# Stanford-ILIAD/PantheonRL

Hardware: AMD Instinct MI355X
Metric: env-steps/sec (all agents) Overcooked-simple PPO self-play (higher is better)
Workload: dtype f32; 1 GPU; OvercookedMultiEnv-v0 layout=simple, PPO self-play (two independent PPO learners per GPU), synthetic (n_envs, n_steps, obs_dim) rollouts; n_envs=1024, n_steps=128, obs_dim=62, features=62, n_logits=6, batch_size=32768, n_epochs=10, agents_per_gpu=2, parallelism=2 agent(s) per gpu x1 gpu(s) = 2 learners (single process), launch_mode=graph, gemm_mode=2, action_masks=none, rollout=scripted, rollout_requested=scripted

## Files before the change

pantheonrl_amd/csrc/ph_abi.hip:

```cpp
#include <dlfcn.h>
#include <hip/hip_runtime.h>
#include <rccl/rccl.h>

#include <atomic>
#include <chrono>
#include <cmath>
#include <cstdio>
#include <cstdint>
#include <cstring>
#include <mutex>
#include <string>
#include <vector>

#include "ph_launch.h"
#include "ph_block.h"
#include "ph_arch.h"
#include "ph_pool.h"

namespace ph {

namespace {
struct LdsGrant {
  const void* kernel;
  int device;
// ... 67 lines not shown
  int* slab_map_split = nullptr;
  int* wimage_map = nullptr;
  int split_kind = 0;
  int slab_len_split = 0;
  int wimage_elems = 0;
  int id = 0;
};

}

struct ph_ctx {
  int device = 0;
  hipStream_t stream = nullptr;
  float* slabs = nullptr;
  size_t slabs_cap = 0;
  float* statpart = nullptr;
  size_t statpart_cap = 0;
  float* grad = nullptr;
  size_t grad_cap = 0;
  float* blocksq = nullptr;
  size_t blocksq_cap = 0;
  float* advstats = nullptr;
  size_t advstats_cap = 0;
  float* act_stage_host = nullptr;
  float* act_stage_dev = nullptr;
  size_t act_stage_cap = 0;
  unsigned int* act_done_host = nullptr;
  unsigned int* act_done_dev = nullptr;
  unsigned int act_seq = 0;
  unsigned int* fwd_host_done = nullptr;
  int joint_reward_rule = 0;
  int wimage_zeroed_for = 0;
  size_t wimage_cap = 0;
  bool exclusive = false;
  unsigned short* wimage = nullptr;
  double* advpart = nullptr;
  size_t advpart_cap = 0;
  int* perm_idx = nullptr;
  size_t perm_idx_cap = 0;
  int* perm_phys = nullptr;
  size_t perm_phys_cap = 0;
  uint4* ximg = nullptr;
  size_t ximg_cap = 0;
  uint4* rec_pi = nullptr;
  uint4* rec_vf = nullptr;
  size_t rec_cap = 0;
// ... 540 lines not shown
    return fail("hipMalloc(ctx scalars) failed");
  }
  (void)hipMemset(c->scalars, 0, 4 * sizeof(float));
  (void)hipMemset(c->stop_flag, 0, sizeof(int));
  (void)hipEventCreate(&c->ev0);
  (void)hipEventCreate(&c->ev1);
  *out = c;
  return 0;
}

int ph_ctx_destroy(ph_ctx* ctx) {
  DevGuard dev_guard(ctx);
  if (!ctx) return 0;
  (void)hipStreamSynchronize(ctx->stream);
  for (auto g : ctx->graphs)
    if (g) (void)hipGraphExecDestroy(g);
  for (auto& s : ctx->specs) {
    if (s.obs_off) (void)hipFree(s.obs_off);
    if (s.slab_map) (void)hipFree(s.slab_map);
    if (s.slab_map_split) (void)hipFree(s.slab_map_split);
    if (s.wimage_map) (void)hipFree(s.wimage_map);
    if (s.act_off) (void)hipFree(s.act_off);
  }
  void* ptrs[] = {ctx->wimage, ctx->mw.act, ctx->mw.maps, ctx->mw.kl_sum, ctx->mw.scratch, ctx->advpart, ctx->p2p_dev, ctx->slabs, ctx->statpart, ctx->grad, ctx->blocksq, ctx->advstats, ctx->perm_idx, ctx->perm_phys, ctx->ximg, ctx->rec_pi, ctx->rec_vf, ctx->rowrec, ctx->step_words, ctx->step_gen, ctx->scalars, ctx->stop_flag,
                  ctx->adap_extra, ctx->adap_loss, ctx->am_buf, ctx->pool_dev, ctx->pool_order, ctx->pool_tiles};
  for (void* p : ptrs)
    if (p) (void)hipFree(p);
  if (ctx->act_stage_host) (void)hipHostFree(ctx->act_stage_host);
  if (ctx->act_done_host) (void)hipHostFree(ctx->act_done_host);
  if (ctx->ev0) (void)hipEventDestroy(ctx->ev0);
  if (ctx->ev1) (void)hipEventDestroy(ctx->ev1);
  if (ctx->ev_grad) (void)hipEventDestroy(ctx->ev_grad);
  (void)ph_comm_destroy(ctx);
  delete ctx;
  return 0;
}

int ph_ctx_set_joint_reward_rule(ph_ctx* ctx, int rule) {
  if (!ctx) return fail("null ctx");
  if (rule != PH_JOINT_MATCH_BONUS && rule != PH_JOINT_RPS) return fail("ph_ctx_set_joint_reward_rule: unknown rule");
  ctx->joint_reward_rule = rule;
  return 0;
}

int ph_ctx_set_stream(ph_ctx* ctx, void* hip_stream) {
  DevGuard dev_guard(ctx);
  if (!ctx) return fail("null ctx");
// ... 1418 lines not shown
  aa.rec_vf_out = nd.split == 1 ? ctx->rec_vf : nullptr;
  aa.rowrec = (nd.split == 1 && rb->advantages && rb->log_probs && rb->actions && rb->returns && rb->values) ? ctx->rowrec : nullptr;
  aa.rb_logp = rb->log_probs;
  aa.rb_act = rb->actions;
  aa.rb_ret = rb->returns;
  aa.rb_val = rb->values;
}


void select_gemm(ph::NetDims& nd, int gemm_mode) {
  nd.split = (gemm_mode == 2 && nd.slab_map_split != nullptr) ? nd.split_kind : 0;
  if (nd.split) nd.slab_map = nd.slab_map_split;
}

int slab_len_of(const ph::NetDims& nd) { return nd.split ? nd.slab_len_split : (nd.slab_map ? 2 * ph::RS_NET : nd.lay.P); }

int ensure_train_ws(ph_ctx* ctx, int P, int slab_len, int nwg_max, int n_mb_total, size_t n_idx = 0, size_t n_phys = 0) {
  if (n_phys && ensure(ctx, ctx->perm_phys, ctx->perm_phys_cap, n_phys)) return 1;
  if (ensure(ctx, ctx->slabs, ctx->slabs_cap, (size_t)nwg_max * slab_len)) return 1;
  if (ensure(ctx, ctx->statpart, ctx->statpart_cap, (size_t)2 * nwg_max * ph::NSTATP)) return 1;
  if (ensure(ctx, ctx->grad, ctx->grad_cap, (size_t)P)) return 1;
  if (ensure(ctx, ctx->blocksq, ctx->blocksq_cap, (size_t)ph::reduce_blocks(slab_len))) return 1;
  if (ensure(ctx, ctx->advstats, ctx->advstats_cap, (size_t)n_mb_total * 2)) return 1;
  if (ensure(ctx, ctx->advpart, ctx->advpart_cap, (size_t)n_mb_total * 2 * ph::ADV_SPLIT)) return 1;
  if (n_idx && ensure(ctx, ctx->perm_idx, ctx->perm_idx_cap, n_idx)) return 1;
  const size_t n_words = (size_t)ph::reduce_blocks(slab_len) + 1;
  if (n_words > ctx->step_words_cap) {
    if (ensure(ctx, ctx->step_words, ctx->step_words_cap, n_words)) return 1;
    PH_HIP(hipMemsetAsync(ctx->step_words, 0, n_words * sizeof(unsigned long long), ctx->stream));
  }
  if (!ctx->step_gen) {
    if (ctx->capturing) return fail("workspace would grow inside graph capture: run the same call once outside capture first");
    PH_HIP(hipMalloc((void**)&ctx->step_gen, 4 * sizeof(unsigned int)));
    PH_HIP(hipMemsetAsync(ctx->step_gen, 0, 4 * sizeof(unsigned int), ctx->stream));
  }
  return 0;
}

bool step_fused_wanted(const ph_ctx* ctx, int slab_len, bool alone) {
  return alone && ctx->exclusive && ctx->step_words && ctx->step_gen &&
         ph::step_fused_fits(ph::reduce_blocks(slab_len), slab_len, ctx->num_cu);
}

}

namespace {
// ... 63 lines not shown
  a.used_state_idx = ad->used_state_idx ? ad->used_state_idx + (size_t)mbi * S : nullptr;
  a.used_contexts = ad->used_contexts ? ad->used_contexts + (size_t)mbi * C * cs : nullptr;
  a.stop_flag = ctx->stop_flag;
  a.prof = ctx->prof;
  PH_HIP(ph::launch_adap_context(a, nwg, ctx->stream));
  r->extra = ctx->adap_extra;
  r->n_extra = nwg;
  r->extra_len = ph::adap_slab_floats(nd.lay);
  r->extra_cut = nd.lay.vf_W1;
  r->extra_lo = nd.lay.act_W;
  r->extra_hi = nd.lay.val_W;
  r->extra_loss = ctx->adap_loss;
  r->extra_norm = 1.0f / (float)((C * (C - 1) / 2) * n_states);
  r->extra_coef = ad->context_loss_coeff;
  r->extra_loss_out = ad->context_loss ? ad->context_loss + mbi : nullptr;
  return 0;
}

void train_adv_args(const TrainPlan& t, bool need_idx, ph::AdvStatArgs& aa) {
  aa = adv_args_epochs(t.ctx, t.rb, t.perms, t.perm_seed, t.batch_size, t.n_mb);
  aa.clear_flag = t.ctx->stop_flag;
  if (t.nd.split == 1 && !need_idx) aa.idx_out = aa.phys_out = nullptr;
  fill_adv_records(aa, t.ctx, t.nd, t.rb);
}

int train_prepare(const char* who, TrainPlan& t, ph_ctx* ctx, const ph_spec* spec, const ph_opt_state* opt, const ph_rollout* rb,
                  const ph_ppo_hyper* hp, int n_epochs, int batch_size, const int* perms, unsigned long long perm_seed,
                  float* stats, int gemm_mode, bool need_idx = false, const ph_arch* arch = nullptr) {
  if (check_train_call(who, ctx, opt, hp, n_epochs, batch_size) || check_rb(rb)) return 1;
  t.arch = arch != nullptr;
  if (arch) {
    if (arch_resolve(ctx, spec, arch, &t.nd, &t.arch_dims)) return 1;
  } else {
    if (resolve(ctx, spec, &t.nd, true)) return 1;
    select_gemm(t.nd, gemm_mode);
  }
  t.ctx = ctx;
  t.opt = opt;
  t.rb = rb;
  t.hp = hp;
  t.perms = perms;
  t.perm_seed = perm_seed;
  t.stats = stats;
  t.n_epochs = n_epochs;
  t.batch_size = batch_size;
  t.gemm_mode = gemm_mode;
// ... 32 lines not shown
    g.rec_vf = ctx->rec_vf + pos;
  }
  g.perm_n = (uint32_t)t.N;
  g.perm_hb = t.hb;
  g.perm_seed = t.perm_seed;
  g.perm_epoch = w.ep;
  g.epoch = ctx->rng_epoch;
  g.mb_start = w.start;
  g.nb = w.nb;
  g.advstats = ctx->advstats + 2 * (size_t)mbi;
  g.ntiles = pl.ntiles;
  *pl_out = pl;
  if (t.arch) PH_HIP(ph::launch_arch_grad(g, t.arch_dims, pl.nwg, t.gemm_mode, ctx->stream));
  else PH_HIP(ph::launch_ppo_grad(g, pl.nwg, t.gemm_mode, ctx->stream));
  return 0;
}

void fill_step_args(const TrainPlan& t, int mbi, const MbPlan& pl, ph::ReduceArgs& r, ph::AdamArgs& ad) {
  ph_ctx* ctx = t.ctx;
  float* stats_out = t.stats ? t.stats + (size_t)mbi * PH_NSTAT : nullptr;
  r = reduce_args(ctx, t.hp, t.opt, t.P, slab_len_of(t.nd), t.nd.slab_map, pl.nwg, pl.nb, ctx->grad, stats_out);
  r.wide = t.alone && ctx->exclusive;
  ad = adam_args(ctx, t.hp, t.opt, t.P, slab_len_of(t.nd), stats_out, t.nd.split ? ctx->wimage : nullptr, t.nd.wimage_map);
}

int train_launch_step(const TrainPlan& t, int mbi, const MbPlan& pl) {
  ph_ctx* ctx = t.ctx;
  hipStream_t s = ctx->stream;
  ph::ReduceArgs r;
  ph::AdamArgs ad;
  fill_step_args(t, mbi, pl, r, ad);
  if (t.adap) {
    const MbWalk w = minibatch_walk(ctx, t.perms, t.N, t.n_mb, t.batch_size, mbi);
    if (adap_launch(ctx, t.nd, t.opt->params, t.rb, t.adap, w.idx, w.nb, mbi, &r)) return 1;
  }
  if (step_fused_wanted(ctx, slab_len_of(t.nd), t.alone != 0)) {
    PH_HIP(ph::launch_ppo_step(r, ad, ctx->step_words, ctx->step_gen, ctx->step_gen + 1, STEP_WAIT_TICKS, s));
  } else {
    PH_HIP(ph::launch_ppo_reduce(r, s));
    PH_HIP(ph::launch_ppo_adam(ad, s));
  }
  return 0;
}

}

// ... 483 lines not shown
  auto timed = [&](int slot, auto&& fn) -> int {
    float ms = 0.f;
    if (time_reps(ctx, 1, reps, [&](int) { return fn(); }, &ms)) return 1;
    us_out[slot] = 1e3f * ms;
    return 0;
  };
  auto hip = [](hipError_t e) { return hip_rc(e, "ph_bench_train_kernels"); };
  if (t.nd.split) {
    if (timed(PH_BENCH_WEIGHT_IMAGE, [&] { return rebuild_weight_image(ctx, t.nd, opt->params); })) return 1;
    if (timed(PH_BENCH_OBS_PLANES, [&] { return build_grad_pack(ctx, t.nd, rb, (size_t)n_epochs * t.N); })) return 1;
  }
  ph::AdvStatArgs aa;
  train_adv_args(t, false, aa);
  if (timed(PH_BENCH_ADV_STATS, [&] { return hip(ph::launch_adv_stats(aa, n_epochs * t.n_mb, s)); })) return 1;
  MbPlan pl;
  if (train_launch_grad(t, 0, &pl)) return 1;
  ph::ReduceArgs r;
  ph::AdamArgs ad;
  fill_step_args(t, 0, pl, r, ad);
  r.wide = 0;
  if (timed(PH_BENCH_REDUCE, [&] { return hip(ph::launch_ppo_reduce(r, s)); })) return 1;
  r.wide = 1;
  if (timed(PH_BENCH_REDUCE_WIDE, [&] { return hip(ph::launch_ppo_reduce(r, s)); })) return 1;
  if (timed(PH_BENCH_ADAM, [&] { return hip(ph::launch_ppo_adam(ad, s)); })) return 1;
  if (ctx->step_words && ctx->step_gen && ph::step_fused_fits(ph::reduce_blocks(slab_len_of(t.nd)), slab_len_of(t.nd), ctx->num_cu)) {
    if (timed(PH_BENCH_STEP_FUSED, [&] {
          return hip(ph::launch_ppo_step(r, ad, ctx->step_words, ctx->step_gen, ctx->step_gen + 1, STEP_WAIT_TICKS, s));
        }))
      return 1;
  }
  if (rb->T >= 2) {
    const size_t E = (size_t)rb->E;
    if (timed(PH_BENCH_BUFFER_ADD, [&] {
          return hip(ph::launch_buffer_add(rb->observations + E * t.nd.D, rb->actions + E * t.nd.A, rb->rewards + E,
                                           rb->episode_starts + E, rb->values + E, rb->log_probs + E, rb->observations,
                                           rb->actions, rb->episode_starts, rb->values, rb->log_probs, rb->E, t.nd.D, t.nd.A, s));
        }))
      return 1;
  }
  us_out[PH_BENCH_SLAB_FLOATS] = (float)((double)pl.nwg * slab_len_of(t.nd));
  return 0;
}


namespace {

// ... 531 lines not shown
```

pantheonrl_amd/csrc/ph_launch.h:

```cpp
#pragma once
#include "ph_device.h"

namespace ph {

__host__ __device__ inline unsigned p2p_stamp32(unsigned long long epoch, int T, int t) {
  return (unsigned)(epoch * (unsigned long long)T + (unsigned long long)t + 1ull);
}

__device__ __forceinline__ void p2p_note_timeout(unsigned long long* error, int kind, int t, unsigned long long index,
                                                 unsigned long long want, unsigned long long seen) {
  if (atomicAdd(error, 1ull) == 0ull) {
    error[1] = (unsigned long long)(unsigned)kind | ((unsigned long long)(unsigned)(t & 0xffffff) << 8) | (index << 32);
    error[2] = want;
    error[3] = seen;
  }
}

__device__ __forceinline__ void poll_backoff(int& polls) {
  if (polls < 16) __builtin_amdgcn_s_sleep(2);
  else if (polls < 64) __builtin_amdgcn_s_sleep(16);
  else __builtin_amdgcn_s_sleep(127);
  ++polls;
}

// ... 117 lines not shown

__device__ __host__ inline uint64_t epoch_key(uint64_t seed, int epoch) {
  uint64_t z = seed + 0x9E3779B97F4A7C15ull * (uint64_t)(epoch + 1);
  z = (z ^ (z >> 30)) * 0xBF58476D1CE4E5B9ull;
  z = (z ^ (z >> 27)) * 0x94D049BB133111EBull;
  return z ^ (z >> 31);
}

__device__ __forceinline__ int env_major_to_phys(int n, int T, int E) {
  const int e = n / T;
  return (n - e * T) * E + e;
}
__device__ __forceinline__ int minibatch_row(const GradArgs& a, int gi) {
  int n;
  if (a.idx) {
    n = a.idx[gi];
  } else {
    const uint64_t key = epoch_key(a.perm_seed + (a.epoch ? *a.epoch : 0ull), a.perm_epoch);
    n = (int)feistel_perm((uint32_t)(a.mb_start + gi), a.perm_n, a.perm_hb, key);
  }
  return env_major_to_phys(n, a.T, a.E);
}

constexpr int ADV_SPLIT = 32;
constexpr int ADV_THREADS = 256;
struct AdvStatArgs {
  const float* rb_adv;
  int T, E;
  const int* perms;
  uint32_t perm_n, perm_hb;
  uint64_t perm_seed;
  const unsigned long long* epoch;
  int N, batch, n_mb;
  float* out;
  double* partial;
  int* idx_out;
  int* phys_out;
  uint4* rec_pi_out = nullptr;
  uint4* rec_vf_out = nullptr;
  const float *rb_logp = nullptr, *rb_act = nullptr, *rb_ret = nullptr, *rb_val = nullptr;
  const uint4* rowrec = nullptr;
  int* clear_flag = nullptr;
};

struct ReduceArgs {
  const float* slabs;
  int nslab, P;
  int slab_len;
  const int* map;
  float* grad;
  float* blocksq;
  const float* statpart;
  int nstatpart;
  float* stats_out;
  int nb;
  float ent_coef, vf_coef, target_kl;
  int* stop_flag;
  int* step;
  float* scalars;
  const float* extra = nullptr;
  int n_extra = 0, extra_len = 0, extra_cut = 0, extra_lo = 0, extra_hi = 0;
  const float* extra_loss = nullptr;
  float extra_norm = 0.f;
  float extra_coef = 0.f;
  float* extra_loss_out = nullptr;
  int wide = 0;
};

struct AdamArgs {
  float* params;
  float* m;
  float* v;
  const float* grad;
  const float* blocksq;
  int nblk, P;
  const int* step;
  const float* scalars;
  int* stop_flag;
  float lr, beta1, beta2, eps, max_norm;
  float* stats_out;
  unsigned short* wimage;
  const int* wimage_map;
};

struct StepArgs {
  ReduceArgs r;
  AdamArgs ad;
  unsigned long long* words = nullptr;
  unsigned int* gen = nullptr;
  unsigned long long timeout = 0;
  unsigned int* sweep_error = nullptr;
};

size_t fwd_lds_bytes(int R, int Lp);
size_t grad_lds_bytes(int R, int Lp, int onehot_D, int nchunk);
hipError_t launch_policy_fwd(const FwdArgs& a, int gemm_mode, hipStream_t s);
hipError_t launch_policy_fwd_multi(const FwdMulti& m, int n_agents, hipStream_t s);
hipError_t launch_fix_illegal(int* actions, const unsigned char* mask, int n, int L, hipStream_t s);
hipError_t launch_gae(const float* rew, const float* val, const float* es, const float* lv, const float* dn, float* adv,
                      float* ret, int T, int E, double gamma, double lam, int mode, hipStream_t s);
hipError_t launch_buffer_add(float* d_obs, float* d_act, float* d_rew, float* d_es, float* d_val, float* d_lp,
                             const float* obs, const float* act, const float* es, const float* val, const float* lp,
                             int E, int D, int A, hipStream_t s);
hipError_t launch_buffer_compact(const ph_rollout& src, const ph_rollout& dst, const int* cols, int n, int D, int A,
                                 hipStream_t s);
// ... 270 lines not shown
```

pantheonrl_amd/csrc/ph_ppo.hip:

```cpp
#include "ph_launch.h"
#include "ph_split.h"
#include "ph_step.h"

namespace ph {


template <int N>
__device__ __forceinline__ float lds_colsum(const float* p, int stride, float s) {
#pragma unroll
  for (int r0 = 0; r0 < N; r0 += 16) {
    float t[16];
#pragma unroll
    for (int i = 0; i < 16; ++i) t[i] = p[(r0 + i) * stride];
    __builtin_amdgcn_sched_barrier(0);
#pragma unroll
    for (int i = 0; i < 16; ++i) s += t[i];
  }
  return s;
}
template <int N>
__device__ __forceinline__ float lds_coldot(const float* p, int stride, const float* q, int qstride, float s) {
#pragma unroll
  for (int r0 = 0; r0 < N; r0 += 16) {
    float t[16], u[16];
// ... 795 lines not shown
  }
  for (int off = 32; off > 0; off >>= 1) {
    s += __shfl_down(s, off, 64);
    q += __shfl_down(q, off, 64);
  }
  if (lane == 0) {
    sh[0][wave] = s;
    sh[1][wave] = q;
  }
  __syncthreads();
  if (tid == 0) {
    double ts = 0.0, tq = 0.0;
    for (int w = 0; w < ADV_THREADS / 64; ++w) {
      ts += sh[0][w];
      tq += sh[1][w];
    }
    a.partial[((size_t)mb * ADV_SPLIT + seg) * 2 + 0] = ts;
    a.partial[((size_t)mb * ADV_SPLIT + seg) * 2 + 1] = tq;
  }
}
__global__ void adv_finalize_kernel(AdvStatArgs a, int n_total) {
  const int mb = blockIdx.x * blockDim.x + threadIdx.x;
  if (mb >= n_total) return;
  const int k = mb % a.n_mb;
  const int start = k * a.batch;
  const int nb = (a.N - start < a.batch) ? a.N - start : a.batch;
  double ts = 0.0, tq = 0.0;
  for (int seg = 0; seg < ADV_SPLIT; ++seg) {
    ts += a.partial[((size_t)mb * ADV_SPLIT + seg) * 2 + 0];
    tq += a.partial[((size_t)mb * ADV_SPLIT + seg) * 2 + 1];
  }
  const double mean = ts / (double)nb;
  double var = (nb > 1) ? (tq - (double)nb * mean * mean) / (double)(nb - 1) : 0.0;
  if (var < 0.0) var = 0.0;
  a.out[2 * mb + 0] = (float)mean;
  a.out[2 * mb + 1] = (float)sqrt(var);
}
hipError_t launch_adv_stats(const AdvStatArgs& a, int n_total, hipStream_t s) {
  hipLaunchKernelGGL(adv_stats_kernel, dim3(n_total * ADV_SPLIT), dim3(ADV_THREADS), 0, s, a);
  hipLaunchKernelGGL(adv_finalize_kernel, dim3((n_total + 63) / 64), dim3(64), 0, s, a, n_total);
  return hipGetLastError();
}

constexpr int OP_ROWS = 32;
struct RowScalars {
  const float *adv, *logp, *act, *ret, *val;
// ... 32 lines not shown
    pl[0][e] = h;
    pl[1][e] = m;
    pl[2][e] = l;
  }
#pragma unroll
  for (int p = 0; p < 3; ++p) image[row * XIMG_ROW_U4 + p * 8 + g] = __builtin_bit_cast(uint4, pl[p]);
}
hipError_t launch_obs_planes(const float* obs, int n, int D, int F, int fold, uint4* image, const float* adv, const float* logp,
                             const float* act, const float* ret, const float* val, uint4* rowrec, hipStream_t s) {
  const size_t blocks = ((size_t)n + 1 + OP_ROWS - 1) / OP_ROWS;
  RowScalars rs{adv, logp, act, ret, val, (adv && logp && act && ret && val) ? rowrec : nullptr};
  hipLaunchKernelGGL(obs_planes_kernel, dim3((unsigned)blocks), dim3(256), 0, s, obs, n, D, F, fold, image, rs);
  return hipGetLastError();
}

template <int VEC>
__global__ __launch_bounds__(RED_PARAMS * 4) void ppo_reduce_kernel(ReduceArgs a) {
  __shared__ float lds_union[4 * RED_PARAMS];
  static_assert(4 * RED_PARAMS >= 32 * NSTATP + NSTATP || 4 * RED_PARAMS >= 32 * NSTATP, "statistics scratch within the slab scratch");
  float (*gsum)[RED_PARAMS] = reinterpret_cast<float (*)[RED_PARAMS]>(lds_union);
  float (*part)[NSTATP] = reinterpret_cast<float (*)[NSTATP]>(lds_union);
  __shared__ float means[NSTATP];
  const int tid = threadIdx.x;
  if (*a.stop_flag != 0) {
    if (blockIdx.x == 0 && tid < PH_NSTAT && a.stats_out) a.stats_out[tid] = 0.f;
    if (blockIdx.x == 0 && tid == 0) {
      a.scalars[1] = 0.f;
      a.scalars[2] = 0.f;
    }
    return;
  }
  if (blockIdx.x == gridDim.x - 1) {
    (void)reduce_statistics(a, part, means, true);
    return;
  }
  const int dst = reduce_dst(a, blockIdx.x);
  const float g = reduce_positions<VEC>(a, gsum, dst, blockIdx.x);
  if (tid < 64) {
    if (dst >= 0) a.grad[dst] = g;
    float q = g * g;
    for (int off = 32; off > 0; off >>= 1) q += __shfl_down(q, off, 64);
    if (tid == 0) a.blocksq[blockIdx.x] = q;
  }
}

template <int VEC>
__global__ __launch_bounds__(RED_PARAMS * 4) void ppo_step_kernel(StepArgs s) {
  __shared__ float gsum[4][RED_PARAMS];
  __shared__ float part[32][NSTATP];
  __shared__ float means[NSTATP];
  const int nblk = gridDim.x - 1;
  const int stopped = *s.r.stop_flag;
  const unsigned tag = *s.gen + 1u;
  const int step_new = *s.ad.step + 1;
  const unsigned err = *s.sweep_error;
  step_body<VEC>(s, blockIdx.x, nblk, tag, step_new, gsum, part, means, nullptr, stopped, err);
}

int reduce_blocks(int slab_len) { return (slab_len + RED_PARAMS - 1) / RED_PARAMS; }
static int reduce_vec(int slab_len, int exclusive) { return (slab_len % 4 == 0 && exclusive) ? 4 : (slab_len % 2 == 0 ? 2 : 1); }
// ... 21 lines not shown
  s.sweep_error = sweep_error;
  const int nblk = reduce_blocks(r.slab_len);
  if ((unsigned long long)r.nslab * (unsigned long long)r.slab_len * sizeof(float) >= (1ull << 32)) return hipErrorInvalidValue;
  switch (reduce_vec(r.slab_len, 1)) {
    case 4: hipLaunchKernelGGL(ppo_step_kernel<4>, dim3(nblk + 1), dim3(RED_PARAMS * 4), 0, st, s); break;
    case 2: hipLaunchKernelGGL(ppo_step_kernel<2>, dim3(nblk + 1), dim3(RED_PARAMS * 4), 0, st, s); break;
    default: hipLaunchKernelGGL(ppo_step_kernel<1>, dim3(nblk + 1), dim3(RED_PARAMS * 4), 0, st, s); break;
  }
  return hipGetLastError();
}
hipError_t launch_ppo_reduce(const ReduceArgs& a, hipStream_t s) {
  const dim3 grid(reduce_blocks(a.slab_len) + 1), block(RED_PARAMS * 4);
  if ((unsigned long long)a.nslab * (unsigned long long)a.slab_len * sizeof(float) >= (1ull << 32)) return hipErrorInvalidValue;
  switch (reduce_vec(a.slab_len, a.wide)) {
    case 4: hipLaunchKernelGGL(ppo_reduce_kernel<4>, grid, block, 0, s, a); break;
    case 2: hipLaunchKernelGGL(ppo_reduce_kernel<2>, grid, block, 0, s, a); break;
    default: hipLaunchKernelGGL(ppo_reduce_kernel<1>, grid, block, 0, s, a); break;
  }
  return hipGetLastError();
}

__global__ __launch_bounds__(256) void ppo_adam_kernel(AdamArgs a) {
  __shared__ float sh[4];
  __shared__ AdamScalars ks;
  const int tid = threadIdx.x;
  const int p = blockIdx.x * blockDim.x + tid;
  const bool live = p < a.P;
  float gr = 0.f, m0 = 0.f, v0 = 0.f, p0 = 0.f;
  int i0 = -1, i1 = -1;
  if (live) {
    gr = a.grad[p];
    m0 = a.m[p];
    v0 = a.v[p];
    p0 = a.params[p];
    if (a.wimage) {
      i0 = a.wimage_map[2 * p];
      i1 = a.wimage_map[2 * p + 1];
    }
  }
  if (a.scalars[1] == 0.f) {
    if (blockIdx.x == 0 && tid == 0 && a.scalars[2] != 0.f) *a.stop_flag = 1;
    return;
  }
  const int step = (tid == 0) ? *a.step : 0;
  float q = 0.f;
  {
    float x[4];
    for (int k0 = tid; k0 < a.nblk; k0 += 4 * 256) {
#pragma unroll
      for (int u = 0; u < 4; ++u) x[u] = (k0 + 256 * u < a.nblk) ? a.blocksq[k0 + 256 * u] : 0.f;
#pragma unroll
      for (int u = 0; u < 4; ++u)
        if (k0 + 256 * u < a.nblk) q += x[u];
    }
  }
  for (int off = 32; off > 0; off >>= 1) q += __shfl_down(q, off, 64);
  if ((tid & 63) == 0) sh[tid >> 6] = q;
  __syncthreads();
  if (tid == 0) {
    const float total = sqrtf((sh[0] + sh[1]) + (sh[2] + sh[3]));
    ks = adam_scalars(total, a.max_norm, step, a.lr, a.beta1, a.beta2);
    if (blockIdx.x == 0 && a.stats_out) a.stats_out[6] = total;
  }
  __syncthreads();
  if (!live) return;
  const AdamScalars k = ks;
  float m, v;
  const float pn = adam_apply(gr, k, a.beta1, a.beta2, a.eps, m0, v0, p0, &m, &v);
  a.m[p] = m;
  a.v[p] = v;
  a.params[p] = pn;
  if (a.wimage) wimage_put_at(a.wimage, i0, i1, pn);
}

__global__ __launch_bounds__(256) void weight_image_kernel(const float* params, unsigned short* image, const int* map, int P) {
  const int p = blockIdx.x * blockDim.x + threadIdx.x;
  if (p < P) wimage_put(image, map, p, params[p]);
}
__global__ __launch_bounds__(256) void weight_image_check_kernel(const float* params, const unsigned short* image, const int* map, int P,
                                                                 int* mismatches) {
  const int p = blockIdx.x * blockDim.x + threadIdx.x;
  if (p >= P) return;
  __bf16 h, m, l;
  split1(params[p], h, m, l);
  const unsigned short want[3] = {__builtin_bit_cast(unsigned short, h), __builtin_bit_cast(unsigned short, m),
                                  __builtin_bit_cast(unsigned short, l)};
  int bad = 0;
  for (int k = 0; k < 2; ++k) {
    const int pos = map[2 * p + k];
// ... 32 lines not shown
```

pantheonrl_amd/csrc/ph_step.h:

```cpp
#pragma once
#include "ph_launch.h"
#include "ph_split.h"

namespace ph {

constexpr int RED_PARAMS = 64, RED_SUB = 16, RED_SHIFT = 6;

struct AdamScalars {
  float coef, ss, bc2s;
};
__device__ __forceinline__ AdamScalars adam_scalars(float total_norm, float max_norm, int step, float lr, float beta1, float beta2) {
  AdamScalars k;
  const float cc = max_norm / (total_norm + 1e-6f);
  k.coef = cc < 1.0f ? cc : 1.0f;
  const double t = (double)step;
  const double bc1 = 1.0 - pow((double)beta1, t);
  const double bc2 = 1.0 - pow((double)beta2, t);
  k.ss = (float)((double)lr / bc1);
  k.bc2s = (float)sqrt(bc2);
  return k;
}
__device__ __forceinline__ float adam_apply(float grad, const AdamScalars& k, float beta1, float beta2, float eps, float m0, float v0,
                                            float p0, float* m_out, float* v_out) {
#pragma clang fp contract(off)
  const float g = grad * k.coef;
  const float d = g - m0;
  const float m = m0 + d * (1.0f - beta1);
  const float gg = g * g;
  const float v = v0 * beta2 + (1.0f - beta2) * gg;
  const float denom = sqrtf(v) / k.bc2s + eps;
  *m_out = m;
  *v_out = v;
  const float step = k.ss * (m / denom);
  return p0 - step;
}
__device__ __forceinline__ float adam_update(float grad, const AdamScalars& k, float beta1, float beta2, float eps, float* m_p,
                                             float* v_p, float* param_p) {
  float m, v;
  const float pn = adam_apply(grad, k, beta1, beta2, eps, *m_p, *v_p, *param_p, &m, &v);
  *m_p = m;
  *v_p = v;
  *param_p = pn;
  return pn;
}
template <int VEC>
struct RedVec;
template <>
struct RedVec<1> { using T = float; };
template <>
struct RedVec<2> { using T = float2; };
template <>
struct RedVec<4> { using T = float4; };
__device__ __forceinline__ int reduce_dst(const ReduceArgs& a, int blk) {
  const int tid = threadIdx.x;
  if (tid >= RED_PARAMS) return -1;
  const int p = blk * RED_PARAMS + tid;
  return p < a.slab_len ? (a.map ? a.map[p] : p) : -1;
}
template <int VEC, bool COH, typename RSRC>
__device__ __forceinline__ void range_walk(const ReduceArgs& a, const RSRC& rsrc, unsigned stride, int per, bool full, int k0, int p0,
                                           float (&range)[VEC]) {
  using VT = typename RedVec<VEC>::T;
  const int n = (k0 + per <= a.nslab ? per : a.nslab - k0);
  float acc[8][VEC];
#pragma unroll
  for (int u = 0; u < 8; ++u)
#pragma unroll
    for (int c = 0; c < VEC; ++c) acc[u][c] = 0.f;
  if (p0 < a.slab_len) {
    const unsigned lane_off = (unsigned)k0 * stride + (unsigned)p0 * (unsigned)sizeof(float);
    constexpr int AUX = COH ? 16 : 0;
    auto ld = [&](int j) -> VT {
      if constexpr (VEC == 4) return __builtin_bit_cast(VT, __builtin_amdgcn_raw_buffer_load_b128(rsrc, lane_off, (unsigned)j * stride, AUX));
      else if constexpr (VEC == 2) return __builtin_bit_cast(VT, __builtin_amdgcn_raw_buffer_load_b64(rsrc, lane_off, (unsigned)j * stride, AUX));
      else return __builtin_bit_cast(VT, __builtin_amdgcn_raw_buffer_load_b32(rsrc, lane_off, (unsigned)j * stride, AUX));
    };
    auto add = [&](float (&dst)[VEC], const VT& x) {
      const float* xv = reinterpret_cast<const float*>(&x);
#pragma unroll
      for (int c = 0; c < VEC; ++c) dst[c] += xv[c];
    };
// ... 22 lines not shown
#pragma unroll
      for (int u = 0; u < 8; ++u) add(acc[u], x0[u]);
    }
  }
#pragma unroll
  for (int c = 0; c < VEC; ++c)
    range[c] = ((acc[0][c] + acc[1][c]) + (acc[2][c] + acc[3][c])) + ((acc[4][c] + acc[5][c]) + (acc[6][c] + acc[7][c]));
}
__device__ __forceinline__ float extra_terms(const ReduceArgs& a, int dst, float g) {
  if (a.n_extra <= 0) return g;
  const int e = dst < a.extra_cut ? dst : ((dst >= a.extra_lo && dst < a.extra_hi) ? a.extra_cut + (dst - a.extra_lo) : -1);
  if (e < 0) return g;
  for (int k0 = 0; k0 < a.n_extra; k0 += 8) {
    float x[8];
#pragma unroll
    for (int u = 0; u < 8; ++u) x[u] = (k0 + u < a.n_extra) ? a.extra[(size_t)(k0 + u) * a.extra_len + e] : 0.f;
#pragma unroll
    for (int u = 0; u < 8; ++u)
      if (k0 + u < a.n_extra) g += x[u];
  }
  return g;
}
template <int VEC, bool COH = false>
__device__ __forceinline__ float reduce_positions(const ReduceArgs& a, float (*gsum)[RED_PARAMS], int dst, int blk) {
  static_assert(VEC == 1 || VEC == 2 || VEC == 4, "positions per lane");
  constexpr int LP = RED_PARAMS / VEC;
  constexpr int TURNS = 4 / VEC;
  const int tid = threadIdx.x, lane = tid & 63;
  const int wave = __builtin_amdgcn_readfirstlane(tid >> RED_SHIFT);
  const int lp = lane % LP, gw = lane / LP;
  const int p0 = blk * RED_PARAMS + lp * VEC;
  const int per = (a.nslab + RED_SUB - 1) / RED_SUB;
  const bool full = per * RED_SUB == a.nslab;
  const unsigned stride = (unsigned)a.slab_len * (unsigned)sizeof(float);
  const auto rsrc = __builtin_amdgcn_make_buffer_rsrc(const_cast<float*>(a.slabs), 0, (int)((unsigned)a.nslab * stride), 0x00020000);
  float rs[TURNS][VEC];
#pragma unroll
  for (int t = 0; t < TURNS; ++t)
#pragma unroll
    for (int c = 0; c < VEC; ++c) rs[t][c] = 0.f;
#pragma unroll 1
  for (int turn = 0; turn < TURNS; ++turn) {
    const int sub = wave * 4 + gw * TURNS + turn;
    float range[VEC];
    range_walk<VEC, COH>(a, rsrc, stride, per, full, sub * per, p0, range);
#pragma unroll
    for (int c = 0; c < VEC; ++c) {
#pragma unroll
      for (int t = 0; t < TURNS; ++t) rs[t][c] = (turn == t) ? range[c] : rs[t][c];
    }
  }
  {
    float q[VEC];
#pragma unroll
    for (int c = 0; c < VEC; ++c) q[c] = rs[0][c];
#pragma unroll
    for (int g = 0; g < VEC; ++g)
#pragma unroll
      for (int turn = 0; turn < TURNS; ++turn) {
        if (g == 0 && turn == 0) continue;
#pragma unroll
        for (int c = 0; c < VEC; ++c) q[c] += (g == 0) ? rs[turn][c] : __shfl(rs[turn][c], lp + g * LP, 64);
      }
    if (gw == 0) {
#pragma unroll
      for (int c = 0; c < VEC; ++c) gsum[wave][lp * VEC + c] = q[c];
    }
  }
  __syncthreads();
  float g = 0.f;
  if (tid < RED_PARAMS) {
    g = (gsum[0][tid] + gsum[1][tid]) + (gsum[2][tid] + gsum[3][tid]);
    g = dst >= 0 ? extra_terms(a, dst, g) : 0.f;
  }
  return g;
}
template <bool COH = false>
__device__ __forceinline__ bool reduce_statistics(const ReduceArgs& a, float (*part)[NSTATP], float* means, bool bump_step) {
  const int tid = threadIdx.x;
  bool stop = false;
  if (tid < 256) {
    const int kst = tid & (NSTATP - 1), j = tid >> 3;
    float v = 0.f;
    for (int w0 = j; w0 < a.nstatpart; w0 += 32 * 16) {
      float x[16];
#pragma unroll
      for (int u = 0; u < 16; ++u) {
        const int w = w0 + 32 * u;
        x[u] = 0.f;
        if (w < a.nstatpart) {
          if constexpr (COH) x[u] = __hip_atomic_load(a.statpart + (size_t)w * NSTATP + kst, __ATOMIC_RELAXED, __HIP_MEMORY_SCOPE_AGENT);
          else x[u] = a.statpart[(size_t)w * NSTATP + kst];
        }
      }
#pragma unroll
      for (int u = 0; u < 16; ++u)
        if (w0 + 32 * u < a.nstatpart) v += x[u];
    }
    part[j][kst] = v;
  }
  __syncthreads();
  if (tid < NSTATP) {
    float v = 0.f;
    for (int j = 0; j < 32; ++j) v += part[j][tid];
    means[tid] = v / (float)a.nb;
  }
  __syncthreads();
  if (tid == 0) {
    const float pl_ = means[0], vl = means[1], el = means[2], cf = means[3], kl = means[4];
    stop = (a.target_kl >= 0.f) && (kl > 1.5f * a.target_kl);
    if (bump_step && !stop && a.step) *a.step += 1;
    a.scalars[0] = kl;
    a.scalars[1] = stop ? 0.f : 1.f;
    a.scalars[2] = stop ? 1.f : 0.f;
    if (a.stats_out) {
      a.stats_out[0] = pl_;
      a.stats_out[1] = vl;
      a.stats_out[2] = el;
      a.stats_out[3] = cf;
      a.stats_out[4] = kl;
      a.stats_out[5] = pl_ + a.ent_coef * el + a.vf_coef * vl;
      a.stats_out[6] = 0.f;
      a.stats_out[7] = stop ? 0.f : 1.f;
    }
    if (a.n_extra > 0) {
      float raw = 0.f;
      for (int k0 = 0; k0 < a.n_extra; k0 += 16) {
        float x[16];
#pragma unroll
        for (int u = 0; u < 16; ++u) x[u] = (k0 + u < a.n_extra) ? a.extra_loss[k0 + u] : 0.f;
#pragma unroll
        for (int u = 0; u < 16; ++u)
          if (k0 + u < a.n_extra) raw += x[u];
      }
      raw *= a.extra_norm;
      if (a.extra_loss_out) *a.extra_loss_out = raw;
      if (a.stats_out) a.stats_out[5] += a.extra_coef * raw;
    }
  }
  return stop;
}

__device__ __forceinline__ void step_finish(const StepArgs& s, int nblk, unsigned tag, int step_new, int lane, bool first, float g,
                                            int dst, float m0, float v0, float p0, int i0, int i1) {
  const ReduceArgs& a = s.r;
// ... 2 lines not shown
  constexpr int MAXW = 16;
  float qv[MAXW];
  bool ok = false;
  const long long t0 = wall_clock64();
  while (true) {
    bool all = true;
#pragma unroll
    for (int i = 0; i < MAXW; ++i) {
      const int k = lane + 64 * i;
      qv[i] = 0.f;
      if (k <= nblk) {
        const unsigned long long w = __hip_atomic_load(s.words + k, __ATOMIC_RELAXED, __HIP_MEMORY_SCOPE_AGENT);
        all = all && ((unsigned)(w >> 32) == tag);
        qv[i] = __uint_as_float((unsigned)w);
      }
    }
    if (__all(all)) { ok = true; break; }
    if ((unsigned long long)(wall_clock64() - t0) > s.timeout) break;
    __builtin_amdgcn_s_sleep(4);
  }
  if (!ok) {
    if (lane == 0) {
      atomicAdd(s.sweep_error, 1u);
      if (first && a.stats_out) a.stats_out[7] = -1.f;
    }
    return;
  }
  int stop_i = 0;
#pragma unroll
  for (int i = 0; i < MAXW; ++i)
    if (lane + 64 * i == nblk) stop_i = __float_as_int(qv[i]) & 1;
  const bool stop = __any(stop_i != 0);
  float shv[4];
#pragma unroll
  for (int v = 0; v < 4; ++v) {
    float q = 0.f;
#pragma unroll
    for (int i = v; i < MAXW; i += 4)
      if (lane + 64 * i < nblk) q += qv[i];
    for (int off = 32; off > 0; off >>= 1) q += __shfl_down(q, off, 64);
    shv[v] = __shfl(q, 0, 64);
  }
  const float total = sqrtf((shv[0] + shv[1]) + (shv[2] + shv[3]));
  if (first && lane == 0) {
    if (!stop && ad.step) *const_cast<int*>(ad.step) = step_new;
    if (stop) *a.stop_flag = 1;
    *s.gen = tag;
    if (!stop && a.stats_out) a.stats_out[6] = total;
  }
  if (stop || dst < 0) return;
  {
    const float cc = ad.max_norm / (total + 1e-6f);
    k.coef = cc < 1.0f ? cc : 1.0f;
  }
  const int p = dst;
  float m, v;
  const float pn = adam_apply(g, k, ad.beta1, ad.beta2, ad.eps, m0, v0, p0, &m, &v);
  ad.m[p] = m;
  ad.v[p] = v;
  ad.params[p] = pn;
  if (ad.wimage) wimage_put_at(ad.wimage, i0, i1, pn);
}


__device__ __forceinline__ void step_stopped(const ReduceArgs& a) {
  const int tid = threadIdx.x;
  if (tid < PH_NSTAT && a.stats_out) a.stats_out[tid] = 0.f;
  if (tid == 0) {
    a.scalars[1] = 0.f;
    a.scalars[2] = 0.f;
  }
}
__device__ __forceinline__ bool step_refused(const ReduceArgs& a, int blk, int stopped, unsigned err) {
  if (err != 0u) {
    if (blk == 0 && threadIdx.x == 0 && a.stats_out) a.stats_out[7] = -1.f;
    return true;
  }
  if (stopped != 0) {
    if (blk == 0) step_stopped(a);
    return true;
  }
  return false;
}
template <int VEC, bool COH = false>
__device__ __forceinline__ void step_body(const StepArgs& s, int blk, int nblk, unsigned tag, int step_new, float (*gsum)[RED_PARAMS],
                                          float (*part)[NSTATP], float* means, const void* , int stopped = 0, unsigned err = 0u) {
  const ReduceArgs& a = s.r;
  const AdamArgs& ad = s.ad;
  const int tid = threadIdx.x;
  if (blk == nblk) {
    if (step_refused(a, blk, stopped, err)) return;
    const bool stop = reduce_statistics<COH>(a, part, means, false);
    if (tid == 0)
      __hip_atomic_store(s.words + nblk, ((unsigned long long)tag << 32) | (stop ? 1ull : 0ull), __ATOMIC_RELAXED, __HIP_MEMORY_SCOPE_AGENT);
    return;
  }
  const int dst = reduce_dst(a, blk);
  float m0 = 0.f, v0 = 0.f, p0 = 0.f;
  int i0 = -1, i1 = -1;
  if (dst >= 0) {
    m0 = ad.m[dst];
    v0 = ad.v[dst];
    p0 = ad.params[dst];
    if (ad.wimage) {
      i0 = ad.wimage_map[2 * dst];
      i1 = ad.wimage_map[2 * dst + 1];
    }
  }
  const float g = reduce_positions<VEC, COH>(a, gsum, dst, blk);
  if (step_refused(a, blk, stopped, err)) return;
  if (tid < 64) {
    float q = g * g;
    for (int off = 32; off > 0; off >>= 1) q += __shfl_down(q, off, 64);
    if (tid == 0)
      __hip_atomic_store(s.words + blk, ((unsigned long long)tag << 32) | (unsigned long long)__float_as_uint(q), __ATOMIC_RELAXED,
// ... 11 lines not shown
```

Measured before the change: 123.5 million agent-steps/s.

## Precompute Adam bias-correction scalars and overlap stop-flag checks with loads

Moves the per-step Adam bias-correction computation, which uses double-precision pow and sqrt, into the advantage-finalize kernel. It writes one AdamBias record per minibatch, and the Adam kernel reads it when the step matches and otherwise recomputes. The Adam kernel drops a shared-memory broadcast and a __syncthreads, and issues its stop-flag and step reads as uniform atomic loads early. The reduce kernel now issues map fetches and the quarter reductions before checking the stop flag, hiding that latency at the cost of wasted work when stopped. Stats handling for the norm slot is adjusted to stay consistent.

```diff
diff --git a/pantheonrl_amd/csrc/ph_abi.hip b/pantheonrl_amd/csrc/ph_abi.hip
--- a/pantheonrl_amd/csrc/ph_abi.hip
+++ b/pantheonrl_amd/csrc/ph_abi.hip
@@ -113,6 +113,8 @@
   size_t blocksq_cap = 0;
   float* advstats = nullptr;
   size_t advstats_cap = 0;
+  ph::AdamBias* adam_bias = nullptr;
+  size_t adam_bias_cap = 0;
   float* act_stage_host = nullptr;
   float* act_stage_dev = nullptr;
   size_t act_stage_cap = 0;
@@ -699,7 +701,7 @@
     if (s.wimage_map) (void)hipFree(s.wimage_map);
     if (s.act_off) (void)hipFree(s.act_off);
   }
-  void* ptrs[] = {ctx->wimage, ctx->mw.act, ctx->mw.maps, ctx->mw.kl_sum, ctx->mw.scratch, ctx->advpart, ctx->p2p_dev, ctx->slabs, ctx->statpart, ctx->grad, ctx->blocksq, ctx->advstats, ctx->perm_idx, ctx->perm_phys, ctx->ximg, ctx->rec_pi, ctx->rec_vf, ctx->rowrec, ctx->step_words, ctx->step_gen, ctx->scalars, ctx->stop_flag,
+  void* ptrs[] = {ctx->wimage, ctx->mw.act, ctx->mw.maps, ctx->mw.kl_sum, ctx->mw.scratch, ctx->advpart, ctx->p2p_dev, ctx->slabs, ctx->statpart, ctx->grad, ctx->blocksq, ctx->advstats, ctx->adam_bias, ctx->perm_idx, ctx->perm_phys, ctx->ximg, ctx->rec_pi, ctx->rec_vf, ctx->rowrec, ctx->step_words, ctx->step_gen, ctx->scalars, ctx->stop_flag,
                   ctx->adap_extra, ctx->adap_loss, ctx->am_buf, ctx->pool_dev, ctx->pool_order, ctx->pool_tiles};
   for (void* p : ptrs)
     if (p) (void)hipFree(p);
@@ -2164,6 +2166,7 @@
   if (ensure(ctx, ctx->grad, ctx->grad_cap, (size_t)P)) return 1;
   if (ensure(ctx, ctx->blocksq, ctx->blocksq_cap, (size_t)ph::reduce_blocks(slab_len))) return 1;
   if (ensure(ctx, ctx->advstats, ctx->advstats_cap, (size_t)n_mb_total * 2)) return 1;
+  if (ensure(ctx, ctx->adam_bias, ctx->adam_bias_cap, (size_t)n_mb_total)) return 1;
   if (ensure(ctx, ctx->advpart, ctx->advpart_cap, (size_t)n_mb_total * 2 * ph::ADV_SPLIT)) return 1;
   if (n_idx && ensure(ctx, ctx->perm_idx, ctx->perm_idx_cap, n_idx)) return 1;
   const size_t n_words = (size_t)ph::reduce_blocks(slab_len) + 1;
@@ -2273,6 +2276,11 @@
   aa.clear_flag = t.ctx->stop_flag;
   if (t.nd.split == 1 && !need_idx) aa.idx_out = aa.phys_out = nullptr;
   fill_adv_records(aa, t.ctx, t.nd, t.rb);
+  aa.adam_bias = t.ctx->adam_bias;
+  aa.opt_step = t.opt->step;
+  aa.lr = t.hp->learning_rate;
+  aa.beta1 = t.hp->adam_beta1;
+  aa.beta2 = t.hp->adam_beta2;
 }
 
 int train_prepare(const char* who, TrainPlan& t, ph_ctx* ctx, const ph_spec* spec, const ph_opt_state* opt, const ph_rollout* rb,
@@ -2351,6 +2359,7 @@
   r = reduce_args(ctx, t.hp, t.opt, t.P, slab_len_of(t.nd), t.nd.slab_map, pl.nwg, pl.nb, ctx->grad, stats_out);
   r.wide = t.alone && ctx->exclusive;
   ad = adam_args(ctx, t.hp, t.opt, t.P, slab_len_of(t.nd), stats_out, t.nd.split ? ctx->wimage : nullptr, t.nd.wimage_map);
+  ad.bias = ctx->adam_bias + mbi;
 }
 
 int train_launch_step(const TrainPlan& t, int mbi, const MbPlan& pl) {
@@ -2880,6 +2889,7 @@
   if (timed(PH_BENCH_REDUCE, [&] { return hip(ph::launch_ppo_reduce(r, s)); })) return 1;
   r.wide = 1;
   if (timed(PH_BENCH_REDUCE_WIDE, [&] { return hip(ph::launch_ppo_reduce(r, s)); })) return 1;
+  if (hip(ph::launch_adv_stats(aa, n_epochs * t.n_mb, s)) || hip(ph::launch_ppo_reduce(r, s))) return 1;
   if (timed(PH_BENCH_ADAM, [&] { return hip(ph::launch_ppo_adam(ad, s)); })) return 1;
   if (ctx->step_words && ctx->step_gen && ph::step_fused_fits(ph::reduce_blocks(slab_len_of(t.nd)), slab_len_of(t.nd), ctx->num_cu)) {
     if (timed(PH_BENCH_STEP_FUSED, [&] {
diff --git a/pantheonrl_amd/csrc/ph_launch.h b/pantheonrl_amd/csrc/ph_launch.h
--- a/pantheonrl_amd/csrc/ph_launch.h
+++ b/pantheonrl_amd/csrc/ph_launch.h
@@ -163,6 +163,12 @@
   return env_major_to_phys(n, a.T, a.E);
 }
 
+struct alignas(16) AdamBias {
+  float ss, bc2s;
+  int step;
+  int pad;
+};
+
 constexpr int ADV_SPLIT = 32;
 constexpr int ADV_THREADS = 256;
 struct AdvStatArgs {
@@ -182,6 +188,9 @@
   const float *rb_logp = nullptr, *rb_act = nullptr, *rb_ret = nullptr, *rb_val = nullptr;
   const uint4* rowrec = nullptr;
   int* clear_flag = nullptr;
+  AdamBias* adam_bias = nullptr;
+  const int* opt_step = nullptr;
+  float lr = 0.f, beta1 = 0.f, beta2 = 0.f;
 };
 
 struct ReduceArgs {
@@ -222,6 +231,7 @@
   float* stats_out;
   unsigned short* wimage;
   const int* wimage_map;
+  const AdamBias* bias = nullptr;
 };
 
 struct StepArgs {
diff --git a/pantheonrl_amd/csrc/ph_ppo.hip b/pantheonrl_amd/csrc/ph_ppo.hip
--- a/pantheonrl_amd/csrc/ph_ppo.hip
+++ b/pantheonrl_amd/csrc/ph_ppo.hip
@@ -841,6 +841,13 @@
 __global__ void adv_finalize_kernel(AdvStatArgs a, int n_total) {
   const int mb = blockIdx.x * blockDim.x + threadIdx.x;
   if (mb >= n_total) return;
+  if (a.adam_bias) {
+    AdamBias b;
+    b.step = *a.opt_step + 1 + mb;
+    b.pad = 0;
+    adam_step_scalars(b.step, a.lr, a.beta1, a.beta2, &b.ss, &b.bc2s);
+    a.adam_bias[mb] = b;
+  }
   const int k = mb % a.n_mb;
   const int start = k * a.batch;
   const int nb = (a.N - start < a.batch) ? a.N - start : a.batch;
@@ -919,20 +926,19 @@
   float (*part)[NSTATP] = reinterpret_cast<float (*)[NSTATP]>(lds_union);
   __shared__ float means[NSTATP];
   const int tid = threadIdx.x;
-  if (*a.stop_flag != 0) {
-    if (blockIdx.x == 0 && tid < PH_NSTAT && a.stats_out) a.stats_out[tid] = 0.f;
-    if (blockIdx.x == 0 && tid == 0) {
-      a.scalars[1] = 0.f;
-      a.scalars[2] = 0.f;
-    }
+  const int stop_word = uniform_word(a.stop_flag);
+  if (blockIdx.x == gridDim.x - 1) {
+    if (__builtin_amdgcn_readfirstlane(stop_word) == 0) (void)reduce_statistics(a, part, means, true);
     return;
   }
-  if (blockIdx.x == gridDim.x - 1) {
-    (void)reduce_statistics(a, part, means, true);
+  const int fetched = reduce_dst_fetch(a, blockIdx.x);
+  reduce_quarters<VEC>(a, gsum, blockIdx.x);
+  if (__builtin_amdgcn_readfirstlane(stop_word) != 0) {
+    if (blockIdx.x == 0) step_stopped(a);
     return;
   }
-  const int dst = reduce_dst(a, blockIdx.x);
-  const float g = reduce_positions<VEC>(a, gsum, dst, blockIdx.x);
+  const int dst = reduce_dst_select(a, blockIdx.x, fetched);
+  const float g = reduce_fold(a, gsum, dst);
   if (tid < 64) {
     if (dst >= 0) a.grad[dst] = g;
     float q = g * g;
@@ -1000,7 +1006,6 @@
 
 __global__ __launch_bounds__(256) void ppo_adam_kernel(AdamArgs a) {
   __shared__ float sh[4];
-  __shared__ AdamScalars ks;
   const int tid = threadIdx.x;
   const int p = blockIdx.x * blockDim.x + tid;
   const bool live = p < a.P;
@@ -1016,11 +1021,14 @@
       i1 = a.wimage_map[2 * p + 1];
     }
   }
-  if (a.scalars[1] == 0.f) {
-    if (blockIdx.x == 0 && tid == 0 && a.scalars[2] != 0.f) *a.stop_flag = 1;
-    return;
-  }
-  const int step = (tid == 0) ? *a.step : 0;
+  const float applied_w = uniform_word(a.scalars + 1);
+  const int step_w = uniform_word(a.step);
+  unsigned long long b0 = 0ull, b1 = 0ull;
+  if (a.bias) {
+    const unsigned long long* bw = reinterpret_cast<const unsigned long long*>(a.bias);
+    b0 = uniform_word(bw);
+    b1 = uniform_word(bw + 1);
+  }
   float q = 0.f;
   {
     float x[4];
@@ -1032,17 +1040,26 @@
         if (k0 + 256 * u < a.nblk) q += x[u];
     }
   }
+  const float applied = __builtin_bit_cast(float, __builtin_amdgcn_readfirstlane(__builtin_bit_cast(int, applied_w)));
+  if (applied == 0.f) {
+    if (blockIdx.x == 0 && tid == 0 && a.scalars[2] != 0.f) *a.stop_flag = 1;
+    return;
+  }
+  const int step = __builtin_amdgcn_readfirstlane(step_w);
+  AdamScalars k;
+  if (a.bias && __builtin_amdgcn_readfirstlane((int)(unsigned)b1) == step) {
+    k.ss = __uint_as_float((unsigned)b0);
+    k.bc2s = __uint_as_float((unsigned)(b0 >> 32));
+  } else {
+    adam_step_scalars(step, a.lr, a.beta1, a.beta2, &k.ss, &k.bc2s);
+  }
   for (int off = 32; off > 0; off >>= 1) q += __shfl_down(q, off, 64);
   if ((tid & 63) == 0) sh[tid >> 6] = q;
   __syncthreads();
-  if (tid == 0) {
-    const float total = sqrtf((sh[0] + sh[1]) + (sh[2] + sh[3]));
-    ks = adam_scalars(total, a.max_norm, step, a.lr, a.beta1, a.beta2);
-    if (blockIdx.x == 0 && a.stats_out) a.stats_out[6] = total;
-  }
-  __syncthreads();
+  const float total = sqrtf((sh[0] + sh[1]) + (sh[2] + sh[3]));
+  k.coef = adam_clip_coef(total, a.max_norm);
+  if (blockIdx.x == 0 && tid == 0 && a.stats_out) a.stats_out[6] = total;
   if (!live) return;
-  const AdamScalars k = ks;
   float m, v;
   const float pn = adam_apply(gr, k, a.beta1, a.beta2, a.eps, m0, v0, p0, &m, &v);
   a.m[p] = m;
diff --git a/pantheonrl_amd/csrc/ph_step.h b/pantheonrl_amd/csrc/ph_step.h
--- a/pantheonrl_amd/csrc/ph_step.h
+++ b/pantheonrl_amd/csrc/ph_step.h
@@ -6,18 +6,29 @@
 
 constexpr int RED_PARAMS = 64, RED_SUB = 16, RED_SHIFT = 6;
 
+template <typename T>
+__device__ __forceinline__ T uniform_word(const T* p) {
+  return __hip_atomic_load(p, __ATOMIC_RELAXED, __HIP_MEMORY_SCOPE_AGENT);
+}
+
 struct AdamScalars {
   float coef, ss, bc2s;
 };
-__device__ __forceinline__ AdamScalars adam_scalars(float total_norm, float max_norm, int step, float lr, float beta1, float beta2) {
-  AdamScalars k;
-  const float cc = max_norm / (total_norm + 1e-6f);
-  k.coef = cc < 1.0f ? cc : 1.0f;
+__device__ __forceinline__ void adam_step_scalars(int step, float lr, float beta1, float beta2, float* ss, float* bc2s) {
   const double t = (double)step;
   const double bc1 = 1.0 - pow((double)beta1, t);
   const double bc2 = 1.0 - pow((double)beta2, t);
-  k.ss = (float)((double)lr / bc1);
-  k.bc2s = (float)sqrt(bc2);
+  *ss = (float)((double)lr / bc1);
+  *bc2s = (float)sqrt(bc2);
+}
+__device__ __forceinline__ float adam_clip_coef(float total_norm, float max_norm) {
+  const float cc = max_norm / (total_norm + 1e-6f);
+  return cc < 1.0f ? cc : 1.0f;
+}
+__device__ __forceinline__ AdamScalars adam_scalars(float total_norm, float max_norm, int step, float lr, float beta1, float beta2) {
+  AdamScalars k;
+  k.coef = adam_clip_coef(total_norm, max_norm);
+  adam_step_scalars(step, lr, beta1, beta2, &k.ss, &k.bc2s);
   return k;
 }
 __device__ __forceinline__ float adam_apply(float grad, const AdamScalars& k, float beta1, float beta2, float eps, float m0, float v0,
@@ -57,6 +68,15 @@
   const int p = blk * RED_PARAMS + tid;
   return p < a.slab_len ? (a.map ? a.map[p] : p) : -1;
 }
+__device__ __forceinline__ int reduce_dst_fetch(const ReduceArgs& a, int blk) {
+  const int p = blk * RED_PARAMS + ((int)threadIdx.x & (RED_PARAMS - 1));
+  const int pc = p < a.slab_len ? p : a.slab_len - 1;
+  return a.map ? a.map[pc] : pc;
+}
+__device__ __forceinline__ int reduce_dst_select(const ReduceArgs& a, int blk, int fetched) {
+  const int tid = threadIdx.x;
+  return (tid < RED_PARAMS && blk * RED_PARAMS + tid < a.slab_len) ? fetched : -1;
+}
 template <int VEC, bool COH, typename RSRC>
 __device__ __forceinline__ void range_walk(const ReduceArgs& a, const RSRC& rsrc, unsigned stride, int per, bool full, int k0, int p0,
                                            float (&range)[VEC]) {
@@ -125,7 +145,7 @@
   return g;
 }
 template <int VEC, bool COH = false>
-__device__ __forceinline__ float reduce_positions(const ReduceArgs& a, float (*gsum)[RED_PARAMS], int dst, int blk) {
+__device__ __forceinline__ void reduce_quarters(const ReduceArgs& a, float (*gsum)[RED_PARAMS], int blk) {
   static_assert(VEC == 1 || VEC == 2 || VEC == 4, "positions per lane");
   constexpr int LP = RED_PARAMS / VEC;
   constexpr int TURNS = 4 / VEC;
@@ -171,6 +191,9 @@
     }
   }
   __syncthreads();
+}
+__device__ __forceinline__ float reduce_fold(const ReduceArgs& a, float (*gsum)[RED_PARAMS], int dst) {
+  const int tid = threadIdx.x;
   float g = 0.f;
   if (tid < RED_PARAMS) {
     g = (gsum[0][tid] + gsum[1][tid]) + (gsum[2][tid] + gsum[3][tid]);
@@ -178,8 +201,14 @@
   }
   return g;
 }
+template <int VEC, bool COH = false>
+__device__ __forceinline__ float reduce_positions(const ReduceArgs& a, float (*gsum)[RED_PARAMS], int dst, int blk) {
+  reduce_quarters<VEC, COH>(a, gsum, blk);
+  return reduce_fold(a, gsum, dst);
+}
 template <bool COH = false>
-__device__ __forceinline__ bool reduce_statistics(const ReduceArgs& a, float (*part)[NSTATP], float* means, bool bump_step) {
+__device__ __forceinline__ bool reduce_statistics(const ReduceArgs& a, float (*part)[NSTATP], float* means, bool bump_step,
+                                                  bool zero_norm = true) {
   const int tid = threadIdx.x;
   bool stop = false;
   if (tid < 256) {
@@ -223,7 +252,7 @@
       a.stats_out[3] = cf;
       a.stats_out[4] = kl;
       a.stats_out[5] = pl_ + a.ent_coef * el + a.vf_coef * vl;
-      a.stats_out[6] = 0.f;
+      if (zero_norm) a.stats_out[6] = 0.f;
       a.stats_out[7] = stop ? 0.f : 1.f;
     }
     if (a.n_extra > 0) {
@@ -272,7 +301,10 @@
   if (!ok) {
     if (lane == 0) {
       atomicAdd(s.sweep_error, 1u);
-      if (first && a.stats_out) a.stats_out[7] = -1.f;
+      if (first && a.stats_out) {
+        a.stats_out[6] = 0.f;
+        a.stats_out[7] = -1.f;
+      }
     }
     return;
   }
@@ -296,7 +328,7 @@
     if (!stop && ad.step) *const_cast<int*>(ad.step) = step_new;
     if (stop) *a.stop_flag = 1;
     *s.gen = tag;
-    if (!stop && a.stats_out) a.stats_out[6] = total;
+    if (a.stats_out) a.stats_out[6] = stop ? 0.f : total;
   }
   if (stop || dst < 0) return;
   {
@@ -340,7 +372,7 @@
   const int tid = threadIdx.x;
   if (blk == nblk) {
     if (step_refused(a, blk, stopped, err)) return;
-    const bool stop = reduce_statistics<COH>(a, part, means, false);
+    const bool stop = reduce_statistics<COH>(a, part, means, false, false);
     if (tid == 0)
       __hip_atomic_store(s.words + nblk, ((unsigned long long)tag << 32) | (stop ? 1ull : 0ull), __ATOMIC_RELAXED, __HIP_MEMORY_SCOPE_AGENT);
     return;
```

Result: faster. 126.0 million agent-steps/s, median of 6 (+2.0%).
